# westlake-moonlight/vision_transformer_detector

Hardware: AMD Instinct MI355X
Metric: images/sec ViT-B/16 detector fwd, batch 256, 1/2/4/8 MI355X; MFMA util % (higher is better)
Workload: dtype bf16; 1 GPU; vit_b16_224 detector forward + decode; per_gpu_batch=256, global_batch=256, parallelism=dp1, streams_per_gpu=2, hip_graph=False

## Files before the change

### vision_transformer_detector_amd/csrc/vtd_gemm.hip

```cpp
#include <stdlib.h>

#include <algorithm>
#include <mutex>
#include <type_traits>

#include "vtd_common.h"
#include "vtd_gemm_epi.h"
#include "vtd_launch.h"

namespace vtd {

namespace {

constexpr int BM = 128, BN = 128, KB = 128;
constexpr int NT = 256;
constexpr int TILE_BYTES = BM * KB;


__device__ __forceinline__ int swz(int row, int chunk) {
  return row * KB + ((chunk ^ (row & 7)) << 4);
}


__device__ __forceinline__ void gload4(i32x4 (&ra)[4], i32x4 (&rb)[4], const char* ga,
                                       const char* gb, const int64_t (&offa)[4],
                                       const int64_t (&offb)[4], int kt, int aw) {
  const int64_t o = (int64_t)kt * KB, oa = (int64_t)(kt >= aw ? kt - aw : kt) * KB;
#pragma unroll
  for (int i = 0; i < 4; ++i) {
    ra[i] = *reinterpret_cast<const i32x4*>(ga + offa[i] + oa);
    rb[i] = *reinterpret_cast<const i32x4*>(gb + offb[i] + o);
  }
}
__device__ __forceinline__ void swrite4(const i32x4 (&ra)[4], const i32x4 (&rb)[4],
                                        char* lds_a, char* lds_b, int srow, int schunk,
                                        int buf) {
#pragma unroll
  for (int i = 0; i < 4; ++i) {
    const int o = buf * TILE_BYTES + swz(srow + 32 * i, schunk);
    *reinterpret_cast<i32x4*>(lds_a + o) = ra[i];
    *reinterpret_cast<i32x4*>(lds_b + o) = rb[i];
  }
}


template <typename T>
__global__ __launch_bounds__(NT) void gemm_tn_kernel(
    int M, int N, int K, const T* __restrict__ A, int lda, const T* __restrict__ Bt,
    int ldb, EpiArgs e) {
  extern __shared__ __attribute__((aligned(16))) char smem[];
  char* lds_a = smem;
  char* lds_b = smem + 2 * TILE_BYTES;

  const int tid = threadIdx.x;
  const int lane = tid & 63, wave = tid >> 6;
  const int wm = wave >> 1, wn = wave & 1;
  const int m0 = blockIdx.y * BM, n0 = blockIdx.x * BN;

  const int srow = tid >> 3, schunk = tid & 7;
  const char* ga = reinterpret_cast<const char*>(A) + schunk * 16;
  const char* gb = reinterpret_cast<const char*>(Bt) + schunk * 16;
  const int64_t lda_b = (int64_t)lda * sizeof(T), ldb_b = (int64_t)ldb * sizeof(T);
  int64_t offa[4], offb[4];
#pragma unroll
  for (int i = 0; i < 4; ++i) {
    offa[i] = (int64_t)min(m0 + srow + 32 * i, M - 1) * lda_b;
    offb[i] = (int64_t)min(n0 + srow + 32 * i, N - 1) * ldb_b;
  }
  i32x4 ra_[4], rb_[4];

  f32x4 acc[4][4];
#pragma unroll
  for (int i = 0; i < 4; ++i)
#pragma unroll
    for (int j = 0; j < 4; ++j) acc[i][j] = f32x4{0.f, 0.f, 0.f, 0.f};

  const int fr = lane & 15, fg = lane >> 4;
  const int nk = K * (int)sizeof(T) / KB;

  gload4(ra_, rb_, ga, gb, offa, offb, 0, e.aw);
  swrite4(ra_, rb_, lds_a, lds_b, srow, schunk, 0);
  __syncthreads();

  for (int kt = 0; kt < nk; ++kt) {
    const int buf = kt & 1;
    if (kt + 1 < nk) gload4(ra_, rb_, ga, gb, offa, offb, kt + 1, e.aw);
    const char* la = lds_a + buf * TILE_BYTES;
    const char* lb = lds_b + buf * TILE_BYTES;
#pragma unroll
    for (int s = 0; s < 2; ++s) {
      const int c = 4 * s + fg;
      i32x4 af[4], bfr[4];
#pragma unroll
      for (int i = 0; i < 4; ++i) {
        af[i] = *reinterpret_cast<const i32x4*>(la + swz(wm * 64 + i * 16 + fr, c));
        bfr[i] = *reinterpret_cast<const i32x4*>(lb + swz(wn * 64 + i * 16 + fr, c));
      }
#pragma unroll
      for (int i = 0; i < 4; ++i)
#pragma unroll
        for (int j = 0; j < 4; ++j) {
          if constexpr (sizeof(T) == 2) {
            acc[i][j] = __builtin_amdgcn_mfma_f32_16x16x32_bf16(
                __builtin_bit_cast(bf16x8, af[i]), __builtin_bit_cast(bf16x8, bfr[j]),
                acc[i][j], 0, 0, 0);
          } else {
            const f32x4 a4 = __builtin_bit_cast(f32x4, af[i]);
            const f32x4 b4 = __builtin_bit_cast(f32x4, bfr[j]);
#pragma unroll
            for (int t = 0; t < 4; ++t)
              acc[i][j] = __builtin_amdgcn_mfma_f32_16x16x4f32(a4[t], b4[t], acc[i][j],
                                                                0, 0, 0);
          }
        }
    }
    if (kt + 1 < nk) swrite4(ra_, rb_, lds_a, lds_b, srow, schunk, buf ^ 1);
    __syncthreads();
  }

#pragma unroll
  for (int i = 0; i < 4; ++i)
#pragma unroll
    for (int j = 0; j < 4; ++j)
#pragma unroll
      for (int r = 0; r < 4; ++r) {
        int m = m0 + wm * 64 + i * 16 + fg * 4 + r;
        int n = n0 + wn * 64 + j * 16 + fr;
        epi_store(e, M, N, m, n, acc[i][j][r]);
      }
}

constexpr int SK_ROWS = 64, SK_CH = 8, SK_KMAX = 2048;
__global__ __launch_bounds__(256) void gemm_skinny_kernel(int M, int N, int K,
                                                          const bf16_t* __restrict__ A, int lda,
                                                          const bf16_t* __restrict__ Bt, int ldb,
                                                          EpiArgs e) {
  extern __shared__ __attribute__((aligned(16))) char smem[];
  const int tid = threadIdx.x, lane = tid & 63, wave = tid >> 6;
  const int fr = lane & 15, g = lane >> 4;
  const int m0 = blockIdx.x * SK_ROWS + wave * 16, n0 = blockIdx.y * 32;
  const int nks = K >> 5;
  const bf16_t* ap = A + (int64_t)min(m0 + fr, M - 1) * lda + 8 * g;
  i32x4 a0[SK_CH], a1[SK_CH];
  const int aw2 = 2 * e.aw;
  auto load = [&](i32x4 (&a)[SK_CH], int s0) {
#pragma unroll
    for (int j = 0; j < SK_CH; ++j) {
      const int sa = min(s0 + j, nks - 1);
      a[j] = *reinterpret_cast<const i32x4*>(ap + (sa >= aw2 ? sa - aw2 : sa) * 32);
    }
  };
  load(a0, 0);
  {
    const int bo = e.aw * 32;
    const int kc = (K - bo) >> 3, nch = 32 * kc;
    const int dr = 256 / kc, dc = 256 - dr * kc;
    int r0 = tid / kc, c0 = tid - r0 * kc;
    for (int i0 = tid; i0 < nch; i0 += 8 * 256) {
      i32x4 v[8];
      int rr[8], cc[8];
#pragma unroll
      for (int u = 0; u < 8; ++u) {
        rr[u] = r0;
        cc[u] = c0;
        v[u] = i32x4{0, 0, 0, 0};
        if (i0 + u * 256 < nch && n0 + r0 < N)
          v[u] = *reinterpret_cast<const i32x4*>(Bt + (int64_t)(n0 + r0) * ldb + bo + c0 * 8);
        r0 += dr;
        c0 += dc;
        if (c0 >= kc) {
          c0 -= kc;
          ++r0;
        }
      }
#pragma unroll
      for (int u = 0; u < 8; ++u)
        if (i0 + u * 256 < nch) {
          const int r = rr[u], t = cc[u] >> 3, c = cc[u] & 7;
          *reinterpret_cast<i32x4*>(smem + t * 4096 + r * 128 + ((c ^ (r & 7)) << 4)) = v[u];
        }
    }
  }
  __syncthreads();
  f32x4 acc[2] = {f32x4{0.f, 0.f, 0.f, 0.f}, f32x4{0.f, 0.f, 0.f, 0.f}};
  auto compute = [&](const i32x4 (&a)[SK_CH], int s0) {
#pragma unroll
    for (int j = 0; j < SK_CH; ++j) {
      const int st = s0 + j;
      if (st < nks) {
        const int sb = st >= e.aw ? st - e.aw : st;
#pragma unroll
        for (int cb = 0; cb < 2; ++cb) {
          const int r = 16 * cb + fr, c = 4 * (sb & 1) + g;
          const bf16x8 b = *reinterpret_cast<const bf16x8*>(smem + (sb >> 1) * 4096 + r * 128 +
                                                            ((c ^ (r & 7)) << 4));
          acc[cb] = __builtin_amdgcn_mfma_f32_16x16x32_bf16(__builtin_bit_cast(bf16x8, a[j]), b,
                                                            acc[cb], 0, 0, 0);
        }
      }
    }
  };
  for (int s0 = 0; s0 < nks; s0 += 2 * SK_CH) {
    if (s0 + SK_CH < nks) load(a1, s0 + SK_CH);
    compute(a0, s0);
    if (s0 + 2 * SK_CH < nks) load(a0, s0 + 2 * SK_CH);
    if (s0 + SK_CH < nks) compute(a1, s0 + SK_CH);
  }
#pragma unroll
  for (int cb = 0; cb < 2; ++cb)
#pragma unroll
    for (int r = 0; r < 4; ++r) epi_store(e, M, N, m0 + 4 * g + r, n0 + 16 * cb + fr, acc[cb][r]);
}

constexpr int BBM = 256, BBN = 256, BNT = 512;
#ifndef VTD_TRS
#define VTD_TRS 0
#endif
#ifndef VTD_PP2_PH
#define VTD_PP2_PH 2
#endif
constexpr int BSTAGE = (BBM + BBN) * KB;
static_assert(8 * 32 * 68 * 4 + 8 * 128 * 8 <= 2 * BSTAGE,
              "epilogue staging + LayerNorm-fold row tables must fit the stages");

typedef __attribute__((address_space(3))) void lds_void_t;
typedef __attribute__((address_space(1))) const void gbl_void_t;


struct NoPF {
  __device__ void operator()() const {}
};

template <int O0, int O1, int O2, int O3>
__device__ __forceinline__ void lds_read4_b64(const void* p, float2 (&o)[4]) {
  const uint32_t a = static_cast<uint32_t>(reinterpret_cast<uintptr_t>(p));
  asm volatile(
      "ds_read_b64 %0, %4 offset:%5\n\tds_read_b64 %1, %4 offset:%6\n\t"
      "ds_read_b64 %2, %4 offset:%7\n\tds_read_b64 %3, %4 offset:%8\n\ts_waitcnt lgkmcnt(0)"
      : "=v"(o[0]), "=v"(o[1]), "=v"(o[2]), "=v"(o[3])
      : "v"(a), "i"(O0), "i"(O1), "i"(O2), "i"(O3)
      : "memory");
}
__device__ __forceinline__ void store_s3(const EpiArgs& e, int64_t idx, const i32x4& o, f32x4 v0,
                                         f32x4 v1) {
  const i32x4 lo = {(int)pack_lo_bf16x2(v0[0], v0[1], (uint32_t)o[0]),
                    (int)pack_lo_bf16x2(v0[2], v0[3], (uint32_t)o[1]),
                    (int)pack_lo_bf16x2(v1[0], v1[1], (uint32_t)o[2]),
                    (int)pack_lo_bf16x2(v1[2], v1[3], (uint32_t)o[3])};
  bf16_t* p = static_cast<bf16_t*>(e.out) + idx;
  store_out16(p + e.s3, lo);
}
template <int EPI, int PR = 32, int DG = 0, typename PF = NoPF, bool TRL = false>
__device__ __forceinline__ void epilogue_fast(const f32x4 (&acc)[8][4], float* ep, int lane,
                                              int m_base, int n_base, const EpiArgs& e,
                                              const float2* lst = nullptr, PF pf = PF{}) {
  constexpr int ACT = EPI & 3;
  constexpr bool OUT_BF16 = (EPI & 4) != 0;
  constexpr bool RESID = (EPI & 8) != 0 && !(DG & 2);
  constexpr bool NOBIAS = (EPI & EPI_PARTIAL) != 0;
  constexpr bool LNF = (EPI & EPI_LNF) != 0, STAT = (EPI & EPI_STAT) != 0 && !(DG & 1);
  constexpr bool F8O = (EPI & EPI_F8O) != 0;
  auto sidx = [](int row, int col) { return row * 64 + (((col >> 2) ^ (row & 7)) << 2) + (col & 3); };
  constexpr int NB = PR / 16;
  constexpr int NIT = PR / 8;
  const int fr = lane & 15, fg = lane >> 4;
  const int c8 = (lane & 7) * 8, rsub = lane >> 3;
  f32x4 b0 = {}, b1 = {};
  if constexpr (!NOBIAS) {
    b0 = *reinterpret_cast<const f32x4*>(e.bias + n_base + c8);
    b1 = *reinterpret_cast<const f32x4*>(e.bias + n_base + c8 + 4);
  }
  f32x4 cs0 = {}, cs1 = {};
  if constexpr (LNF) {
    cs0 = *reinterpret_cast<const f32x4*>(e.colsum + n_base + c8);
    cs1 = *reinterpret_cast<const f32x4*>(e.colsum + n_base + c8 + 4);
  }
  constexpr bool RPRE = RESID && OUT_BF16;
  i32x4 rraw[2][NIT];
  auto load_raw = [&](int pp, i32x4 (&dst)[NIT]) {
#pragma unroll
    for (int it = 0; it < NIT; ++it) {
      const int64_t m = m_base + pp * PR + it * 8 + rsub;
      dst[it] = *reinterpret_cast<const i32x4*>(static_cast<const bf16_t*>(e.resid) + m * e.ldr +
                                                n_base + c8);
    }
  };
  if constexpr (RPRE) load_raw(0, rraw[0]);
  else pf();
#pragma unroll
  for (int p = 0; p < 128 / PR; ++p) {
    if constexpr (TRL) {
#pragma unroll
      for (int i = 0; i < NB; ++i)
#pragma unroll
        for (int jj = 0; jj < 4; ++jj)
          *reinterpret_cast<f32x4*>(ep + sidx(i * 16 + fr, 32 * (jj >> 1) + 8 * fg + 4 * (jj & 1))) =
              acc[p * NB + i][jj];
    } else {
#pragma unroll
      for (int i = 0; i < NB; ++i)
#pragma unroll
        for (int j = 0; j < 4; ++j)
#pragma unroll
          for (int r2 = 0; r2 < 4; ++r2)
            ep[sidx(i * 16 + fg * 4 + r2, j * 16 + fr)] = acc[p * NB + i][j][r2];
    }
    if constexpr (RPRE) {
      if (p + 1 < 128 / PR) load_raw(p + 1, rraw[(p + 1) & 1]);
      if (p == 0) pf();
    }
    constexpr bool ASM_ST = LNF && !std::is_same<PF, NoPF>::value;
    float2 stv[4];
    if constexpr (ASM_ST) {
      static_assert(PR == 32, "the fold's table reads assume 32-row passes");
      if (p == 0) lds_read4_b64<0, 64, 128, 192>(lst + rsub, stv);
      else if (p == 1) lds_read4_b64<256, 320, 384, 448>(lst + rsub, stv);
      else if (p == 2) lds_read4_b64<512, 576, 640, 704>(lst + rsub, stv);
      else lds_read4_b64<768, 832, 896, 960>(lst + rsub, stv);
    }
    f32x4 rv[NIT][2];
    [[maybe_unused]] float2 stkeep = float2{0.f, 0.f};
    if constexpr (RESID && !RPRE) {
#pragma unroll
      for (int it = 0; it < NIT; ++it) {
        const int64_t m = m_base + p * PR + it * 8 + rsub;
        load_resid8<OUT_BF16>(e, m * e.ldr + n_base + c8, rv[it][0], rv[it][1]);
      }
    }
#pragma unroll
    for (int it = 0; it < NIT; ++it) {
      const int row = it * 8 + rsub;
      f32x4 v0 = *reinterpret_cast<const f32x4*>(ep + sidx(row, c8));
      f32x4 v1 = *reinterpret_cast<const f32x4*>(ep + sidx(row, c8 + 4));
      if constexpr (ASM_ST) epi_lnfold8_st(stv[it], cs0, cs1, v0, v1);
      else if constexpr (LNF) epi_lnfold8_st(lst[p * PR + row], cs0, cs1, v0, v1);
      v0 += b0;
      v1 += b1;
      if constexpr ((EPI & EPI_RA) != 0) epi_rowadd8(e, m_base + p * PR + row, n_base + c8, v0, v1);
      act_ct8<ACT>(v0, v1);
      if constexpr (RPRE) {
        const i32x4 w = rraw[p & 1][it];
        v0 += bf16x4_to_f32((uint32_t)w[0], (uint32_t)w[1]);
        v1 += bf16x4_to_f32((uint32_t)w[2], (uint32_t)w[3]);
      } else if constexpr (RESID) {
        v0 += rv[it][0];
        v1 += rv[it][1];
      }
      if constexpr ((EPI & EPI_O2) != 0) epi_out2_8(e, m_base + p * PR + row, n_base + c8, v0, v1);
      const int64_t idx = (int64_t)(m_base + p * PR + row) * e.ldo + n_base + c8;
      if constexpr (OUT_BF16) {
        if constexpr (F8O) {
          bf16_round4(v0);
          bf16_round4(v1);
          float am = 0.f;
#pragma unroll
          for (int j = 0; j < 4; ++j) am = fmaxf(am, fmaxf(fabsf(v0[j]), fabsf(v1[j])));
          am = fmaxf(am, dpp_f32<0xB1>(am));
          am = fmaxf(am, dpp_f32<0x4E>(am));
          const int E = mx8_exponent(am);
          const float inv = __uint_as_float((uint32_t)(127 - E) << 23);
          const uint2 qv = {mx8_pack4(v0[0], v0[1], v0[2], v0[3], inv),
                            mx8_pack4(v1[0], v1[1], v1[2], v1[3], inv)};
          *reinterpret_cast<uint2*>(static_cast<uint8_t*>(e.out) + idx) = qv;
          if ((lane & 3) == 0) {
            const int n = n_base + c8, b = n >> 5;
            e.sout[((int64_t)(b >> 2) * e.s_rows + m_base + p * PR + row) * 4 + (b & 3)] =
                (uint8_t)(E + 127);
          }
          continue;
        }
        const i32x4 o = {(int)pack_bf16x2(v0[0], v0[1]), (int)pack_bf16x2(v0[2], v0[3]),
                         (int)pack_bf16x2(v1[0], v1[1]), (int)pack_bf16x2(v1[2], v1[3])};
        if constexpr (DG & 4) asm volatile("" ::"v"(o));
        else store_out16(static_cast<bf16_t*>(e.out) + idx, o);
        if constexpr ((EPI & EPI_S3) != 0) store_s3(e, idx, o, v0, v1);
        if constexpr (STAT) {
          f32x2 pv[4];
          bf16x8_unpack(o, pv);
          const float mean = sum8_dpp(pairs_sum(pv)) * (1.f / 64.f);
          const float m2 = sum8_dpp(pairs_m2(pv, mean));
          if ((lane & 7) == it) stkeep = float2{mean, m2};
        }
      } else {
        float* op = static_cast<float*>(e.out) + idx;
        *reinterpret_cast<f32x4*>(op) = v0;
        *reinterpret_cast<f32x4*>(op + 4) = v1;
      }
    }
    if constexpr (OUT_BF16 && STAT && !F8O) {
      static_assert(NIT <= 8, "one statistics row per lane of an 8-lane group");
      if ((lane & 7) < NIT)
        e.statout[(int64_t)(n_base >> 6) * e.stat_ld + m_base + p * PR + (lane & 7) * 8 + rsub] =
            stkeep;
    }
  }
}
template <int PR = 32>
__device__ __forceinline__ void epilogue_generic_pass(const float* ep, int lane, int M, int N,
                                                      int m_base, int n_base, const EpiArgs& e) {
  constexpr int ES = 68;
#pragma unroll 1
  for (int it = 0; it < PR / 4; ++it) {
    const int row = it * 4 + (lane >> 4), col = (lane & 15) * 4;
    const f32x4 v = *reinterpret_cast<const f32x4*>(ep + row * ES + col);
    epi_store4(e, M, N, m_base + row, n_base + col, v);
  }
}

template <int PR = 32>
__device__ __forceinline__ void epilogue_generic(const f32x4 (&acc)[8][4], float* ep, int lane,
                                                 int M, int N, int m_base, int n_base,
                                                 const EpiArgs& e) {
  constexpr int ES = 68;
  constexpr int NB = PR / 16;
  const int fr = lane & 15, fg = lane >> 4;
#pragma unroll
  for (int p = 0; p < 128 / PR; ++p) {
#pragma unroll
    for (int i = 0; i < NB; ++i)
#pragma unroll
      for (int j = 0; j < 4; ++j)
#pragma unroll
        for (int r2 = 0; r2 < 4; ++r2)
          ep[(i * 16 + fg * 4 + r2) * ES + j * 16 + fr] = acc[p * NB + i][j][r2];
    epilogue_generic_pass<PR>(ep, lane, M, N, m_base + p * PR, n_base, e);
  }
}

__device__ __forceinline__ void pp_barrier() {
  __builtin_amdgcn_sched_barrier(0);
  asm volatile("" ::: "memory");
  __builtin_amdgcn_s_barrier();
  asm volatile("" ::: "memory");
  __builtin_amdgcn_sched_barrier(0);
}

template <int I0, int J0, bool F32 = false>
__device__ __forceinline__ void pp_mfma(f32x4 (&acc)[8][4], const bf16x8 (&a)[4][2],
                                        const bf16x8 (&b)[2][2]) {
  __builtin_amdgcn_s_setprio(1);
  if constexpr (F32) {
#pragma unroll
    for (int s = 0; s < 2; ++s)
#pragma unroll
      for (int t = 0; t < 4; ++t)
#pragma unroll
        for (int i = 0; i < 4; ++i)
#pragma unroll
          for (int j = 0; j < 2; ++j)
            acc[I0 + i][J0 + j] = __builtin_amdgcn_mfma_f32_16x16x4f32(
                __builtin_bit_cast(f32x4, a[i][s])[t], __builtin_bit_cast(f32x4, b[j][s])[t],
                acc[I0 + i][J0 + j], 0, 0, 0);
  } else {
#pragma unroll
    for (int s = 0; s < 2; ++s)
#pragma unroll
      for (int i = 0; i < 4; ++i)
#pragma unroll
        for (int j = 0; j < 2; ++j)
          acc[I0 + i][J0 + j] =
              __builtin_amdgcn_mfma_f32_16x16x32_bf16(a[i][s], b[j][s], acc[I0 + i][J0 + j], 0, 0, 0);
  }
  __builtin_amdgcn_s_setprio(0);
}

__device__ __forceinline__ void pp_load_a(bf16x8 (&a)[4][2], const char* la, int row0, int fr,
                                          int fg) {
#pragma unroll
  for (int i = 0; i < 4; ++i)
#pragma unroll
    for (int s = 0; s < 2; ++s)
      a[i][s] = *reinterpret_cast<const bf16x8*>(la + swz(row0 + i * 16 + fr, 4 * s + fg));
}
__device__ __forceinline__ void pp_load_b(bf16x8 (&b)[2][2], const char* lb, int row0, int fr,
                                          int fg) {
#pragma unroll
  for (int j = 0; j < 2; ++j)
#pragma unroll
    for (int s = 0; s < 2; ++s)
      b[j][s] = *reinterpret_cast<const bf16x8*>(lb + swz(row0 + j * 16 + fr, 4 * s + fg));
}

__device__ __forceinline__ int swz_t(int row, int chunk) {
  return row * KB + ((chunk ^ (row & 7) ^ ((row >> 2) & 4)) << 4);
}
__device__ __forceinline__ int perm_t(int j, int fr) { return 8 * (fr >> 2) + 4 * j + (fr & 3); }

__device__ __forceinline__ void pp_load_b_t(bf16x8 (&b)[2][2], const char* lb, int row0, int fr,
                                            int fg) {
#pragma unroll
  for (int j = 0; j < 2; ++j)
#pragma unroll
    for (int s = 0; s < 2; ++s)
      b[j][s] = *reinterpret_cast<const bf16x8*>(lb + swz_t(row0 + perm_t(j, fr), 4 * s + fg));
}

template <int I0, int J0, bool F32 = false>
__device__ __forceinline__ void pp_mfma_t(f32x4 (&acc)[8][4], const bf16x8 (&a)[4][2],
                                          const bf16x8 (&b)[2][2]) {
  __builtin_amdgcn_s_setprio(1);
  if constexpr (F32) {
#pragma unroll
    for (int s = 0; s < 2; ++s)
#pragma unroll
      for (int t = 0; t < 4; ++t)
#pragma unroll
        for (int i = 0; i < 4; ++i)
#pragma unroll
          for (int j = 0; j < 2; ++j)
            acc[I0 + i][J0 + j] = __builtin_amdgcn_mfma_f32_16x16x4f32(
                __builtin_bit_cast(f32x4, b[j][s])[t], __builtin_bit_cast(f32x4, a[i][s])[t],
                acc[I0 + i][J0 + j], 0, 0, 0);
  } else {
#pragma unroll
    for (int s = 0; s < 2; ++s)
#pragma unroll
      for (int i = 0; i < 4; ++i)
#pragma unroll
        for (int j = 0; j < 2; ++j)
          acc[I0 + i][J0 + j] =
              __builtin_amdgcn_mfma_f32_16x16x32_bf16(b[j][s], a[i][s], acc[I0 + i][J0 + j], 0, 0, 0);
  }
  __builtin_amdgcn_s_setprio(0);
}

__device__ __forceinline__ int grp_tile_row(int g, int gr) {
  return g < 2 ? (gr & 64) * 2 + g * 64 + (gr & 63)
               : (gr >> 5) * 64 + (g - 2) * 32 + (gr & 31);
}

struct PP2BufSrc {
  __amdgpu_buffer_rsrc_t ra, rb;
  int off[4][2];
  int ak0, aw;
};
template <bool AW>
struct PP2Src : PP2BufSrc {};
constexpr bool pp2_wraps(int code) {
  return code == EPI_GENERIC || (code & EPI_S3) != 0 || (code & 4) == 0;
}

template <bool TR, typename T = bf16_t, bool AW = true>
__device__ __forceinline__ void pp2b_sources(PP2Src<AW>& s, const T* A, int lda, int M,
                                             const T* Bt, int ldb, int N, int m0, int n0,
                                             int wave, int lane, int k0 = 0, bool valid = true,
                                             int aw = 0) {
  constexpr int ES = (int)sizeof(T);
  const int ka0 = AW ? 0 : k0;
  const int64_t ra_bytes = (int64_t)(M - m0) * lda * ES - ES * ka0,
                rb_bytes = (int64_t)(N - n0) * ldb * ES - ES * k0;
  s.ak0 = AW ? k0 * ES / 128 : 0;
  s.aw = AW ? aw : 0;
  s.ra = __builtin_amdgcn_make_buffer_rsrc(const_cast<T*>(A + (int64_t)m0 * lda + ka0), 0,
                                           valid ? (int)std::min<int64_t>(ra_bytes, 0x7fffffff) : 0,
                                           0x00020000);
  s.rb = __builtin_amdgcn_make_buffer_rsrc(const_cast<T*>(Bt + (int64_t)n0 * ldb + k0), 0,
                                           valid ? (int)std::min<int64_t>(rb_bytes, 0x7fffffff) : 0,
                                           0x00020000);
  const int prow = lane >> 3, pchunk = (lane & 7) ^ prow;
#pragma unroll
  for (int g = 0; g < 4; ++g)
#pragma unroll
    for (int j = 0; j < 2; ++j) {
      const int tr = grp_tile_row(g, (wave * 2 + j) * 8 + prow);
      const int bchunk = TR ? pchunk ^ ((wave & 1) << 2) : pchunk;
      s.off[g][j] = g < 2 ? min(tr, M - 1 - m0) * lda * ES + pchunk * 16
                          : min(tr, N - 1 - n0) * ldb * ES + bchunk * 16;
    }
}

template <int G, bool AW>
__device__ __forceinline__ void pp2_issue(char* smem, const PP2BufSrc& src, int wave, int kt,
                                          int stage) {
  char* dst = smem + stage * BSTAGE + G * 16384 + wave * 2 * 1024;
  int ks = kt;
  if constexpr (G < 2 && AW) {
    ks += src.ak0;
    ks = ks >= src.aw ? ks - src.aw : ks;
  }
#pragma unroll
  for (int j = 0; j < 2; ++j)
    __builtin_amdgcn_raw_ptr_buffer_load_lds(G < 2 ? src.ra : src.rb,
                                             (lds_void_t*)(dst + j * 1024), 16, src.off[G][j],
                                             ks * 128, 0, 0);
}

template <bool TR, bool F32 = false, bool NB = false, bool AW = true>
__device__ __forceinline__ void pp2_mainloop(f32x4 (&acc)[8][4], char* smem, const PP2Src<AW>& src,
                                             int nk, int wave, int wm, int wn, int fr, int fg,
                                             uint64_t* t_prologue = nullptr, bool pre = false) {
  if (!pre) {
    pp2_issue<0, AW>(smem, src, wave, 0, 0);
    pp2_issue<2, AW>(smem, src, wave, 0, 0);
    pp2_issue<3, AW>(smem, src, wave, 0, 0);
    pp2_issue<1, AW>(smem, src, wave, 0, 0);
  } else {
    pp_barrier();
  }
  if (nk > 1) {
    pp2_issue<0, AW>(smem, src, wave, 1, 1);
    pp2_issue<2, AW>(smem, src, wave, 1, 1);
    pp2_issue<3, AW>(smem, src, wave, 1, 1);
    asm volatile("s_waitcnt vmcnt(6)" ::: "memory");
  } else {
    asm volatile("s_waitcnt vmcnt(0)" ::: "memory");
  }
  pp_barrier();
  if (t_prologue) *t_prologue = __builtin_amdgcn_s_memtime();
  if (wm == 1) pp_barrier();
  const int ra = wm * 64, rb = wn * 32;
  bf16x8 a[4][2], b0[2][2], b1[2][2];
  auto step = [&](int kt, auto t1, auto t2) {
    const char* st = smem + (kt & 1) * BSTAGE;
    constexpr bool n1 = decltype(t1)::value, n2 = decltype(t2)::value;
    pp_load_a(a, st + 0 * 16384, ra, fr, fg);
    if constexpr (TR) pp_load_b_t(b0, st + 2 * 16384, rb, fr, fg);
    else pp_load_b(b0, st + 2 * 16384, rb, fr, fg);
    if constexpr (n1) pp2_issue<1, AW>(smem, src, wave, kt + 1, (kt + 1) & 1);
    if constexpr (n1) asm volatile("s_waitcnt vmcnt(10)" ::: "memory");
    else asm volatile("s_waitcnt vmcnt(0)" ::: "memory");
    if constexpr (!NB) pp_barrier();
    if constexpr (TR) pp_mfma_t<0, 0, F32>(acc, a, b0);
    else pp_mfma<0, 0, F32>(acc, a, b0);
    if constexpr (!NB) pp_barrier();
    if constexpr (TR) pp_load_b_t(b1, st + 3 * 16384, rb, fr, fg);
    else pp_load_b(b1, st + 3 * 16384, rb, fr, fg);
    if constexpr (n1) asm volatile("s_waitcnt vmcnt(8)" ::: "memory");
    else asm volatile("s_waitcnt vmcnt(0)" ::: "memory");
    if constexpr (!NB) pp_barrier();
    if constexpr (TR) pp_mfma_t<0, 2, F32>(acc, a, b1);
    else pp_mfma<0, 2, F32>(acc, a, b1);
    if constexpr (!NB) pp_barrier();
    pp_load_a(a, st + 1 * 16384, ra, fr, fg);
    if constexpr (n2) pp2_issue<0, AW>(smem, src, wave, kt + 2, kt & 1);
    if constexpr (!NB) pp_barrier();
    if constexpr (TR) pp_mfma_t<4, 2, F32>(acc, a, b1);
    else pp_mfma<4, 2, F32>(acc, a, b1);
    if constexpr (!NB) pp_barrier();
    if constexpr (n2) {
      pp2_issue<2, AW>(smem, src, wave, kt + 2, kt & 1);
      pp2_issue<3, AW>(smem, src, wave, kt + 2, kt & 1);
      asm volatile("s_waitcnt vmcnt(10)" ::: "memory");
    } else {
      asm volatile("s_waitcnt vmcnt(0)" ::: "memory");
    }
    if constexpr (!NB) pp_barrier();
    if constexpr (TR) pp_mfma_t<4, 0, F32>(acc, a, b0);
    else pp_mfma<4, 0, F32>(acc, a, b0);
    if constexpr (!NB) pp_barrier();
  };
  int kt = 0;
  for (; kt + 2 < nk; ++kt) step(kt, std::true_type{}, std::true_type{});
  if (kt + 1 < nk) step(kt++, std::true_type{}, std::false_type{});
  step(kt, std::false_type{}, std::false_type{});
  if (wm == 0) pp_barrier();
}

template <int I0, bool TR, bool F32>
__device__ __forceinline__ void pp_mfma32(f32x4 (&acc)[8][4], const bf16x8 (&a)[4][2],
                                          const bf16x8 (&b0)[2][2], const bf16x8 (&b1)[2][2]) {
  if constexpr (TR) {
    pp_mfma_t<I0, 0, F32>(acc, a, b0);
    pp_mfma_t<I0, 2, F32>(acc, a, b1);
  } else {
    pp_mfma<I0, 0, F32>(acc, a, b0);
    pp_mfma<I0, 2, F32>(acc, a, b1);
  }
}

template <bool TR, bool F32 = false, bool AW = true>
__device__ __forceinline__ void pp2_mainloop_2ph(f32x4 (&acc)[8][4], char* smem,
                                                 const PP2Src<AW>& src, int nk, int wave, int wm,
                                                 int wn, int fr, int fg,
                                                 uint64_t* t_prologue = nullptr) {
  pp2_issue<0, AW>(smem, src, wave, 0, 0);
  pp2_issue<2, AW>(smem, src, wave, 0, 0);
  pp2_issue<3, AW>(smem, src, wave, 0, 0);
  pp2_issue<1, AW>(smem, src, wave, 0, 0);
  if (nk > 1) {
    pp2_issue<0, AW>(smem, src, wave, 1, 1);
    pp2_issue<2, AW>(smem, src, wave, 1, 1);
    pp2_issue<3, AW>(smem, src, wave, 1, 1);
    asm volatile("s_waitcnt vmcnt(6)" ::: "memory");
  } else {
    asm volatile("s_waitcnt vmcnt(0)" ::: "memory");
  }
  pp_barrier();
  if (t_prologue) *t_prologue = __builtin_amdgcn_s_memtime();
  if (wm == 1) pp_barrier();
  const int ra = wm * 64, rb = wn * 32;
  bf16x8 a[4][2], b0[2][2], b1[2][2];
  auto step = [&](int kt, auto t1, auto t2) {
    const char* st = smem + (kt & 1) * BSTAGE;
    constexpr bool n1 = decltype(t1)::value, n2 = decltype(t2)::value;
    pp_load_a(a, st + 0 * 16384, ra, fr, fg);
    if constexpr (TR) {
      pp_load_b_t(b0, st + 2 * 16384, rb, fr, fg);
      pp_load_b_t(b1, st + 3 * 16384, rb, fr, fg);
    } else {
      pp_load_b(b0, st + 2 * 16384, rb, fr, fg);
      pp_load_b(b1, st + 3 * 16384, rb, fr, fg);
    }
    if constexpr (n1) {
      pp2_issue<1, AW>(smem, src, wave, kt + 1, (kt + 1) & 1);
      asm volatile("s_waitcnt vmcnt(8)" ::: "memory");
    } else {
      asm volatile("s_waitcnt vmcnt(0)" ::: "memory");
    }
    pp_barrier();
    pp_mfma32<0, TR, F32>(acc, a, b0, b1);
    pp_barrier();
    pp_load_a(a, st + 1 * 16384, ra, fr, fg);
    if constexpr (n2) {
      pp2_issue<0, AW>(smem, src, wave, kt + 2, kt & 1);
      pp2_issue<2, AW>(smem, src, wave, kt + 2, kt & 1);
      pp2_issue<3, AW>(smem, src, wave, kt + 2, kt & 1);
      asm volatile("s_waitcnt vmcnt(8)" ::: "memory");
    } else {
      asm volatile("s_waitcnt vmcnt(0) lgkmcnt(0)" ::: "memory");
    }
    pp_barrier();
    pp_mfma32<4, TR, F32>(acc, a, b0, b1);
    if (n1 || n2 || wm == 0) pp_barrier();
  };
  int kt = 0;
  for (; kt + 2 < nk; ++kt) step(kt, std::true_type{}, std::true_type{});
  if (kt + 1 < nk) step(kt++, std::true_type{}, std::false_type{});
  step(kt, std::false_type{}, std::false_type{});
}

template <int EPI, int DG = 0, typename PF = NoPF>
__device__ __forceinline__ void epilogue_direct(const f32x4 (&acc)[8][4], int lane, int m_base,
                                                int n_base, const EpiArgs& e,
                                                const float2* lst = nullptr, PF pf = PF{}) {
  constexpr int ACT = EPI & 3;
  constexpr bool OUT_BF16 = (EPI & 4) != 0;
  constexpr bool RESID = (EPI & 8) != 0 && !(DG & 2);
  constexpr bool LNF = (EPI & EPI_LNF) != 0, STAT = (EPI & EPI_STAT) != 0 && !(DG & 1);
  constexpr bool F8O = (EPI & EPI_F8O) != 0;
  static_assert(!(F8O && (STAT || (EPI & EPI_S3) != 0)), "MX-fp8 output: no statistics / split");
  const int fr = lane & 15, fg = lane >> 4;
  f32x4 bias[2][2], cs[2][2] = {};
#pragma unroll
  for (int jp = 0; jp < 2; ++jp)
#pragma unroll
    for (int h = 0; h < 2; ++h) {
      bias[jp][h] = *reinterpret_cast<const f32x4*>(e.bias + n_base + 32 * jp + 8 * fg + 4 * h);
      if constexpr (LNF)
        cs[jp][h] = *reinterpret_cast<const f32x4*>(e.colsum + n_base + 32 * jp + 8 * fg + 4 * h);
    }
  constexpr bool RPRE = RESID && OUT_BF16;
  i32x4 rraw[2][4][2];
  auto load_raw = [&](int h0, i32x4 (&dst)[4][2]) {
#pragma unroll
    for (int i = 0; i < 4; ++i)
#pragma unroll
      for (int jp = 0; jp < 2; ++jp)
        dst[i][jp] = *reinterpret_cast<const i32x4*>(
            static_cast<const bf16_t*>(e.resid) + (int64_t)(m_base + 16 * (h0 + i) + fr) * e.ldr +
            n_base + 32 * jp + 8 * fg);
  };
  if constexpr (RPRE) load_raw(0, rraw[0]);
  else pf();
#pragma unroll
  for (int i0 = 0; i0 < 8; i0 += 4) {
    f32x4 rv[4][2][2];
    float2 st[4];
    if constexpr (LNF && !std::is_same<PF, NoPF>::value) {
      if (i0 == 0) lds_read4_b64<0, 128, 256, 384>(lst + fr, st);
      else lds_read4_b64<512, 640, 768, 896>(lst + fr, st);
    } else if constexpr (LNF) {
#pragma unroll
      for (int i = 0; i < 4; ++i) st[i] = lst[16 * (i0 + i) + fr];
    }
    [[maybe_unused]] float2 stkeep = float2{0.f, 0.f};
    if constexpr (RPRE) {
      if (i0 == 0) {
        load_raw(4, rraw[1]);
        pf();
      }
    } else if constexpr (RESID) {
#pragma unroll
      for (int i = 0; i < 4; ++i)
#pragma unroll
        for (int jp = 0; jp < 2; ++jp) {
          load_resid8<OUT_BF16>(e, (int64_t)(m_base + 16 * (i0 + i) + fr) * e.ldr + n_base +
                                       32 * jp + 8 * fg, rv[i][jp][0], rv[i][jp][1]);
        }
    }
#pragma unroll
    for (int i = 0; i < 4; ++i) {
      float tsum = 0.f;
      i32x4 ob[2];
#pragma unroll
      for (int jp = 0; jp < 2; ++jp) {
        f32x4 v0 = acc[i0 + i][2 * jp];
        f32x4 v1 = acc[i0 + i][2 * jp + 1];
        const int mrow = m_base + 16 * (i0 + i) + fr, ncol = n_base + 32 * jp + 8 * fg;
        if constexpr (LNF)
          epi_lnfold8_st(st[i], cs[jp][0], cs[jp][1], v0, v1);
        v0 += bias[jp][0];
        v1 += bias[jp][1];
        if constexpr ((EPI & EPI_RA) != 0) epi_rowadd8(e, mrow, ncol, v0, v1);
        act_ct8<ACT>(v0, v1);
        if constexpr (RPRE) {
          const i32x4 w = rraw[i0 >> 2][i][jp];
          v0 += bf16x4_to_f32((uint32_t)w[0], (uint32_t)w[1]);
          v1 += bf16x4_to_f32((uint32_t)w[2], (uint32_t)w[3]);
        } else if constexpr (RESID) {
          v0 += rv[i][jp][0];
          v1 += rv[i][jp][1];
        }
        if constexpr ((EPI & EPI_O2) != 0) epi_out2_8(e, mrow, ncol, v0, v1);
        const int64_t idx = (int64_t)mrow * e.ldo + ncol;
        if constexpr (F8O) {
          bf16_round4(v0);
          bf16_round4(v1);
          float am = 0.f;
#pragma unroll
          for (int j = 0; j < 4; ++j) am = fmaxf(am, fmaxf(fabsf(v0[j]), fabsf(v1[j])));
          am = xmax32(xmax16(am));
          const int E = mx8_exponent(am);
          const float inv = __uint_as_float((uint32_t)(127 - E) << 23);
          const uint2 qv = {mx8_pack4(v0[0], v0[1], v0[2], v0[3], inv),
                            mx8_pack4(v1[0], v1[1], v1[2], v1[3], inv)};
          *reinterpret_cast<uint2*>(static_cast<uint8_t*>(e.out) + idx) = qv;
          if (fg == 0) {
            const int b = (n_base + 32 * jp) >> 5;
            e.sout[((int64_t)(b >> 2) * e.s_rows + mrow) * 4 + (b & 3)] = (uint8_t)(E + 127);
          }
          continue;
        }
        if constexpr (OUT_BF16) {
          const i32x4 o = {(int)pack_bf16x2(v0[0], v0[1]), (int)pack_bf16x2(v0[2], v0[3]),
                           (int)pack_bf16x2(v1[0], v1[1]), (int)pack_bf16x2(v1[2], v1[3])};
          if constexpr (DG & 4) asm volatile("" ::"v"(o));
          else store_out16(static_cast<bf16_t*>(e.out) + idx, o);
          if constexpr ((EPI & EPI_S3) != 0) store_s3(e, idx, o, v0, v1);
          if constexpr (STAT) {
            ob[jp] = o;
            tsum += bf16x8_sum(o);
          }
        } else {
          float* op = static_cast<float*>(e.out) + idx;
          *reinterpret_cast<f32x4*>(op) = v0;
          *reinterpret_cast<f32x4*>(op + 4) = v1;
        }
      }
      if constexpr (OUT_BF16 && STAT) {
        const float mean = xsum32(xsum16(tsum)) * (1.f / 64.f);
        const float m2 = xsum32(xsum16(bf16x8_m2(ob[0], mean) + bf16x8_m2(ob[1], mean)));
        if (fg == i) stkeep = float2{mean, m2};
      }
    }
    if constexpr (OUT_BF16 && STAT)
      e.statout[(int64_t)(n_base >> 6) * e.stat_ld + m_base + 16 * (i0 + fg) + fr] = stkeep;
  }
}

__device__ __forceinline__ void epilogue_direct_generic(const f32x4 (&acc)[8][4], float* ep,
                                                        int lane, int M, int N, int m_base,
                                                        int n_base, const EpiArgs& e) {
  constexpr int ES = 68;
  const int fr = lane & 15, fg = lane >> 4;
#pragma unroll
  for (int p = 0; p < 4; ++p) {
#pragma unroll
    for (int i = 0; i < 2; ++i)
#pragma unroll
      for (int jj = 0; jj < 4; ++jj)
        *reinterpret_cast<f32x4*>(ep + (i * 16 + fr) * ES + 32 * (jj >> 1) + 8 * fg +
                                  4 * (jj & 1)) = acc[p * 2 + i][jj];
    epilogue_generic_pass<32>(ep, lane, M, N, m_base + p * 32, n_base, e);
  }
}

#if VTD_DIAG
constexpr int kStampSlots = 16384;
__device__ uint64_t g_pp2_stamps[kStampSlots * 6];
#endif

template <int EPI, bool TR = false, int DG = 0>
__global__ __launch_bounds__(BNT) void gemm_tn_bf16_pp2_kernel(
    int M, int N, int K, const bf16_t* __restrict__ A, int lda,
    const bf16_t* __restrict__ Bt, int ldb, int tiles_m, int tiles_n, EpiArgs e, int ksplit) {
  extern __shared__ __attribute__((aligned(16))) char smem[];
  const int tid = threadIdx.x;
  const int lane = tid & 63;
  const int wave = __builtin_amdgcn_readfirstlane(tid >> 6);
  const int wm = wave >> 2, wn = wave & 3;
  const int nt = tiles_m * tiles_n, nwg = nt * ksplit;
  const int bid = blockIdx.x;
#if VTD_DIAG
  if (e.dsl > 0 && bid < 256 && ((bid >> 3) & 1))
    for (int i = 0; i < e.dsl; ++i) __builtin_amdgcn_s_sleep(8);
#endif
  const int xcd = bid & 7, q = nwg >> 3, r = nwg & 7;
  const int v = (xcd < r ? xcd * (q + 1) : r * (q + 1) + (xcd - r) * q) + (bid >> 3);
  const int split = ksplit > 1 ? v / nt : 0, tile = v - split * nt;
  int tm, tn;
  tile_coords(tile, e.to, tm, tn);
  const int m0 = tm * BBM, n0 = tn * BBN;
  const int nk_all = K / 64, nks = ksplit > 1 ? (nk_all + ksplit - 1) / ksplit : nk_all;
  const int k0 = split * nks, nk = min(nks, nk_all - k0);
  if (ksplit > 1) e.out = static_cast<float*>(e.out) + split * e.split_stride;
  PP2Src<pp2_wraps(EPI)> src;
  pp2b_sources<TR>(src, A, lda, M, Bt, ldb, N, m0, n0, wave, lane, k0 * 64, true, e.aw);
  float2 lst[2] = {float2{0.f, 0.f}, float2{0.f, 0.f}};
  if constexpr (EPI != EPI_GENERIC && (EPI & EPI_LNF) != 0) {
    lst[0] = e.lnstat[min(m0 + wm * 128 + lane, M - 1)];
    lst[1] = e.lnstat[min(m0 + wm * 128 + 64 + lane, M - 1)];
  }
  f32x4 acc[8][4];
#pragma unroll
  for (int i = 0; i < 8; ++i)
#pragma unroll
    for (int j = 0; j < 4; ++j) acc[i][j] = f32x4{0.f, 0.f, 0.f, 0.f};
  const int fr = lane & 15, fg = lane >> 4;
  uint64_t ts[4] = {0, 0, 0, 0};
  [[maybe_unused]] uint64_t rt0 = 0;
  if constexpr ((DG & 16) != 0) {
    ts[0] = __builtin_amdgcn_s_memtime();
    rt0 = __builtin_amdgcn_s_memrealtime();
  }
  if constexpr (VTD_PP2_PH == 2 && (DG & 32) == 0)
    pp2_mainloop_2ph<TR>(acc, smem, src, nk, wave, wm, wn, fr, fg, (DG & 16) ? &ts[1] : nullptr);
  else
    pp2_mainloop<TR, false, (DG & 32) != 0>(acc, smem, src, nk, wave, wm, wn, fr, fg,
                                             (DG & 16) ? &ts[1] : nullptr);
  if constexpr ((DG & 16) != 0) ts[2] = __builtin_amdgcn_s_memtime();
  const int m_base = m0 + wm * 128, n_base = n0 + wn * 64;
#if VTD_DIAG
  auto stamp = [&]() {
    if constexpr ((DG & 16) != 0) {
      ts[3] = __builtin_amdgcn_s_memtime();
      if (wave == 0 && lane == 0 && bid < kStampSlots) {
        g_pp2_stamps[bid * 6 + 0] = ts[0];
        g_pp2_stamps[bid * 6 + 1] = ts[1];
        g_pp2_stamps[bid * 6 + 2] = ts[2];
        g_pp2_stamps[bid * 6 + 3] = ts[3];
        g_pp2_stamps[bid * 6 + 4] = rt0;
        g_pp2_stamps[bid * 6 + 5] = __builtin_amdgcn_s_memrealtime();
      }
    }
  };
#else
  auto stamp = [&]() {};
#endif
  float2* const lds_st = reinterpret_cast<float2*>(smem + 8 * 32 * 68 * 4) + wave * 128;
  if constexpr (EPI != EPI_GENERIC && (EPI & EPI_LNF) != 0) {
    lds_st[lane] = lst[0];
    lds_st[64 + lane] = lst[1];
  }
  if constexpr ((DG & 8) != 0) {
#pragma unroll
    for (int i = 0; i < 8; ++i)
#pragma unroll
      for (int j = 0; j < 4; ++j) asm volatile("" ::"v"(acc[i][j]));
    return;
  }
  if constexpr (TR) {
    if constexpr (EPI != EPI_GENERIC) {
      if (m0 + BBM <= M && n0 + BBN <= N) {
        if constexpr (VTD_TRS && (EPI & 4) != 0 && (EPI & EPI_F8O) == 0)
          epilogue_fast<EPI, 32, DG, NoPF, true>(acc, reinterpret_cast<float*>(smem) + wave * 32 * 68,
                                                 lane, m_base, n_base, e, lds_st);
        else
          epilogue_direct<EPI, DG>(acc, lane, m_base, n_base, e, lds_st);
        stamp();
        return;
      }
    }
    epilogue_direct_generic(acc, reinterpret_cast<float*>(smem) + wave * 32 * 68, lane, M, N,
                            m_base, n_base, e);
    return;
  }
  float* ep = reinterpret_cast<float*>(smem) + wave * 32 * 68;
  if constexpr (EPI != EPI_GENERIC) {
    if (m0 + BBM <= M && n0 + BBN <= N) {
      epilogue_fast<EPI, 32, DG>(acc, ep, lane, m_base, n_base, e, lds_st);
      stamp();
      return;
    }
  }
  epilogue_generic(acc, ep, lane, M, N, m_base, n_base, e);
}
// ... 901 lines not shown
```

Baseline: 20580 images/s.

## Add packed bf16 LDS staging epilogue and relax prologue vmcnt wait

Adds a specialized GEMM epilogue for bf16-output, non-residual cases that packs pairs of bf16 values into 32-bit LDS words with a new swizzle. Rows are then reassembled with byte permutes before 16-byte global stores. The aim is to halve LDS staging traffic and bank pressure in the epilogue, with optional LN-fold, row-add and stat computation kept inline. It also loosens the prologue's s_waitcnt from vmcnt(6) to vmcnt(8); if that count does not match the outstanding loads, the first stage could be read before its data has arrived.

Result: no change. 20720 images/s (median of 6 runs) (+0.7%).

```diff
diff --git a/vision_transformer_detector_amd/csrc/vtd_gemm.hip b/vision_transformer_detector_amd/csrc/vtd_gemm.hip
--- a/vision_transformer_detector_amd/csrc/vtd_gemm.hip
+++ b/vision_transformer_detector_amd/csrc/vtd_gemm.hip
@@ -250,10 +250,126 @@
   bf16_t* p = static_cast<bf16_t*>(e.out) + idx;
   store_out16(p + e.s3, lo);
 }
+constexpr bool epi_packed_staging(int code) {
+  return (code & 4) != 0 && (code & (8 | EPI_PARTIAL | EPI_F8O | EPI_O2 | EPI_S3)) == 0;
+}
+__device__ __forceinline__ int packed_sidx(int q, int col) {
+  return q * 64 + (((col >> 2) ^ (5 * ((q >> 1) & 1))) << 2) + (col & 3);
+}
+template <int EPI, int DG, typename PF>
+__device__ __forceinline__ void epilogue_fast_packed(const f32x4 (&acc)[8][4], float* ep, int lane,
+                                                     int m_base, int n_base, const EpiArgs& e,
+                                                     const float2* lst, PF pf) {
+  constexpr int ACT = EPI & 3;
+  constexpr bool LNF = (EPI & EPI_LNF) != 0, STAT = (EPI & EPI_STAT) != 0 && !(DG & 1);
+  constexpr bool RA = (EPI & EPI_RA) != 0;
+  uint32_t* const sp = reinterpret_cast<uint32_t*>(ep);
+  const int fr = lane & 15, fg = lane >> 4;
+  const int c8 = (lane & 7) * 8, rsub = lane >> 3;
+  float bj[4], cj[4] = {0.f, 0.f, 0.f, 0.f};
+  bool raj[4] = {false, false, false, false};
+#pragma unroll
+  for (int j = 0; j < 4; ++j) {
+    const int n = n_base + 16 * j + fr;
+    bj[j] = e.bias[n];
+    if constexpr (LNF) cj[j] = e.colsum[n];
+    if constexpr (RA) raj[j] = n < e.rowadd_ncols;
+  }
+  pf();
+  constexpr bool ASM_ST = LNF && !std::is_same<PF, NoPF>::value;
+#pragma unroll
+  for (int p = 0; p < 4; ++p) {
+#pragma unroll
+    for (int i = 0; i < 2; ++i) {
+      const int lr = p * 32 + i * 16 + 4 * fg;
+      float2 st[4];
+      if constexpr (ASM_ST) {
+#define VTD_PK_ST(B) \
+  if (p * 2 + i == B) lds_read4_b64<B * 128, B * 128 + 8, B * 128 + 16, B * 128 + 24>(lst + 4 * fg, st);
+        VTD_PK_ST(0) VTD_PK_ST(1) VTD_PK_ST(2) VTD_PK_ST(3)
+        VTD_PK_ST(4) VTD_PK_ST(5) VTD_PK_ST(6) VTD_PK_ST(7)
+#undef VTD_PK_ST
+      } else if constexpr (LNF) {
+#pragma unroll
+        for (int r2 = 0; r2 < 4; ++r2) st[r2] = lst[lr + r2];
+      }
+      float ra[4] = {0.f, 0.f, 0.f, 0.f};
+      if constexpr (RA) {
+        int rm = (m_base + lr) % e.rowadd_period;
+#pragma unroll
+        for (int r2 = 0; r2 < 4; ++r2) {
+          ra[r2] = e.rowadd[rm];
+          rm = rm + 1 == e.rowadd_period ? 0 : rm + 1;
+        }
+      }
+#pragma unroll
+      for (int j = 0; j < 4; j += 2) {
+        f32x4 v0 = acc[p * 2 + i][j], v1 = acc[p * 2 + i][j + 1];
+#pragma unroll
+        for (int r2 = 0; r2 < 4; ++r2) {
+          if constexpr (LNF) {
+            v0[r2] = __builtin_fmaf(__builtin_fmaf(-st[r2].x, cj[j], v0[r2]), st[r2].y, bj[j]);
+            v1[r2] = __builtin_fmaf(__builtin_fmaf(-st[r2].x, cj[j + 1], v1[r2]), st[r2].y, bj[j + 1]);
+          } else {
+            v0[r2] += bj[j];
+            v1[r2] += bj[j + 1];
+          }
+          if constexpr (RA) {
+            v0[r2] += raj[j] ? ra[r2] : 0.f;
+            v1[r2] += raj[j + 1] ? ra[r2] : 0.f;
+          }
+        }
+        act_ct8<ACT>(v0, v1);
+        const int q = i * 8 + 2 * fg;
+        sp[packed_sidx(q, j * 16 + fr)] = pack_bf16x2(v0[0], v0[1]);
+        sp[packed_sidx(q + 1, j * 16 + fr)] = pack_bf16x2(v0[2], v0[3]);
+        sp[packed_sidx(q, j * 16 + 16 + fr)] = pack_bf16x2(v1[0], v1[1]);
+        sp[packed_sidx(q + 1, j * 16 + 16 + fr)] = pack_bf16x2(v1[2], v1[3]);
+      }
+    }
+    [[maybe_unused]] float2 stkeep = float2{0.f, 0.f};
+#pragma unroll
+    for (int t = 0; t < 2; ++t) {
+      const int q = t * 8 + rsub;
+      const i32x4 d0 = *reinterpret_cast<const i32x4*>(sp + packed_sidx(q, c8));
+      const i32x4 d1 = *reinterpret_cast<const i32x4*>(sp + packed_sidx(q, c8 + 4));
+#pragma unroll
+      for (int h = 0; h < 2; ++h) {
+        const uint32_t sel = h ? 0x07060302u : 0x05040100u;
+        const i32x4 o = {(int)__builtin_amdgcn_perm((uint32_t)d0[1], (uint32_t)d0[0], sel),
+                         (int)__builtin_amdgcn_perm((uint32_t)d0[3], (uint32_t)d0[2], sel),
+                         (int)__builtin_amdgcn_perm((uint32_t)d1[1], (uint32_t)d1[0], sel),
+                         (int)__builtin_amdgcn_perm((uint32_t)d1[3], (uint32_t)d1[2], sel)};
+        const int row = p * 32 + 2 * q + h;
+        const int64_t idx = (int64_t)(m_base + row) * e.ldo + n_base + c8;
+        if constexpr (DG & 4) asm volatile("" ::"v"(o));
+        else store_out16(static_cast<bf16_t*>(e.out) + idx, o);
+        if constexpr (STAT) {
+          f32x2 pv[4];
+          bf16x8_unpack(o, pv);
+          const float mean = sum8_dpp(pairs_sum(pv)) * (1.f / 64.f);
+          const float m2 = sum8_dpp(pairs_m2(pv, mean));
+          if ((lane & 7) == 2 * t + h) stkeep = float2{mean, m2};
+        }
+      }
+    }
+    if constexpr (STAT) {
+      const int k = lane & 7;
+      if (k < 4)
+        e.statout[(int64_t)(n_base >> 6) * e.stat_ld + m_base + p * 32 + 16 * (k >> 1) + 2 * rsub +
+                  (k & 1)] = stkeep;
+    }
+  }
+}
+
 template <int EPI, int PR = 32, int DG = 0, typename PF = NoPF, bool TRL = false>
 __device__ __forceinline__ void epilogue_fast(const f32x4 (&acc)[8][4], float* ep, int lane,
                                               int m_base, int n_base, const EpiArgs& e,
                                               const float2* lst = nullptr, PF pf = PF{}) {
+  if constexpr (!TRL && PR == 32 && epi_packed_staging(EPI)) {
+    epilogue_fast_packed<EPI, DG, PF>(acc, ep, lane, m_base, n_base, e, lst, pf);
+    return;
+  }
   constexpr int ACT = EPI & 3;
   constexpr bool OUT_BF16 = (EPI & 4) != 0;
   constexpr bool RESID = (EPI & 8) != 0 && !(DG & 2);
@@ -681,7 +797,7 @@
     pp2_issue<0, AW>(smem, src, wave, 1, 1);
     pp2_issue<2, AW>(smem, src, wave, 1, 1);
     pp2_issue<3, AW>(smem, src, wave, 1, 1);
-    asm volatile("s_waitcnt vmcnt(6)" ::: "memory");
+    asm volatile("s_waitcnt vmcnt(8)" ::: "memory");
   } else {
     asm volatile("s_waitcnt vmcnt(0)" ::: "memory");
   }
```
